# dwave-examples/image-generation

Hardware: AMD Instinct MI355X
Metric: DVAE+GRBM train-step images/s (MNIST) at 1/2/4/8 MI355X; loss parity vs CPU (higher is better)
Workload: dtype f32

## Files before the change

### image-generation_amd/csrc/special.hip

```cpp
#include <cstdlib>
#include "kernels.h"
#include "conv.h"

namespace dvg {

typedef float f32x16c __attribute__((ext_vector_type(16)));
__global__ __launch_bounds__(256) void enc_conv0_fwd_kernel(const float* __restrict__ img, int64_t B,
                                                            const float* __restrict__ w, const float* __restrict__ bias,
                                                            float* __restrict__ Y, float* __restrict__ stats_part) {
  __shared__ double red[2 * 4 * 32];
  const int tid = threadIdx.x, lane = tid & 63, wave = tid >> 6, hh = lane >> 5, c = lane & 31;
  float bw[5];
  int dy[5], dx[5];
#pragma unroll
  for (int j = 0; j < 5; ++j) {
    const int t = 2 * j + hh;
    bw[j] = t < 9 ? w[c * 9 + t] : bias[c];
    dy[j] = t < 9 ? t / 3 - 1 : 0;
    dx[j] = t < 9 ? t % 3 - 1 : 0;
  }
  const int64_t tiles = B * 32;
  double s1 = 0.0, s2 = 0.0;
  constexpr int TU = 2;
  for (int64_t t0 = ((int64_t)blockIdx.x * 4 + wave) * TU; t0 < tiles; t0 += (int64_t)gridDim.x * 4 * TU) {
// ... 345 lines not shown
  DVG_LAUNCH(K_BN_FINALIZE, enc_l0_moments_finalize_kernel, dim3(1), dim3(1024), 0, s, (const double*)part, nblk,
             (double)B * 1024.0, w, bias, mom, mean, invstd, rm, rv, nbt);
  return DVG_OK;
}

__global__ __launch_bounds__(320) void enc_l0_combine_kernel(const float* __restrict__ tot, const double* __restrict__ mom,
                                                             const float* __restrict__ wgt, const float* __restrict__ bias,
                                                             const float* __restrict__ mean, const float* __restrict__ gamma,
                                                             const float* __restrict__ invstd, double M,
                                                             float* __restrict__ gw, float* __restrict__ gb,
                                                             float* __restrict__ g_bn_b, float* __restrict__ g_bn_g) {
  const int w = threadIdx.x;
  const int co = w < 288 ? w / 9 : w - 288, t = w < 288 ? w % 9 : 9;
  const float sum_dz = tot[288 + co], sum_dzzh = tot[320 + co];
  const double m1 = (double)sum_dz / M, m2 = (double)sum_dzzh / M;
  const double shift = (double)bias[co] - (double)mean[co];
  double t1, t2 = 0.0;
  if (t < 9) {
    t1 = mom[t];
    for (int u = 0; u < 9; ++u) t2 += (double)wgt[co * 9 + u] * mom[u <= t ? enc_l0_pair_index(u, t) : enc_l0_pair_index(t, u)];
    t2 += shift * mom[t];
  } else {
    t1 = M;
    for (int u = 0; u < 9; ++u) t2 += (double)wgt[co * 9 + u] * mom[u];
    t2 += shift * M;
  }
  t2 *= (double)invstd[co];
  const float v = (float)((double)gamma[co] * (double)invstd[co] * ((double)tot[w] - m1 * t1 - m2 * t2));
  if (w < 288) gw[w] = v;
  else { gb[co] = v; g_bn_b[co] = sum_dz; g_bn_g[co] = sum_dzzh; }
}

int launch_enc_l0_combine(const float* tot, const double* mom, const float* w, const float* bias, const float* mean,
                          const float* gamma, const float* invstd, int64_t B, float* gw, float* gb, float* g_bn_b,
                          float* g_bn_g, hipStream_t s) {
  DVG_LAUNCH(K_MISC, enc_l0_combine_kernel, dim3(1), dim3(320), 0, s, tot, mom, w, bias, mean, gamma, invstd, (double)B * 1024.0,
             gw, gb, g_bn_b, g_bn_g);
  return DVG_OK;
}

typedef float f32x16s __attribute__((ext_vector_type(16)));
__global__ __launch_bounds__(256) void enc_conv0_wgrad_kernel(const float* __restrict__ img, int64_t B,
                                                              const float* __restrict__ dY, float* __restrict__ part) {
  __shared__ float red[4 * 32 * 33];
  const int tid = threadIdx.x, lane = tid & 63, wave = tid >> 6, hh = lane >> 5, c = lane & 31;
  const int64_t P = B * 1024;
  int64_t per = (P + gridDim.x * 4 - 1) / (gridDim.x * 4);
  per = (per + 1) & ~(int64_t)1;
  const int64_t p0 = ((int64_t)blockIdx.x * 4 + wave) * per;
  const int64_t p1 = p0 + per < P ? p0 + per : P;
  const int dy = c < 9 ? c / 3 - 1 : 0, dx = c < 9 ? c % 3 - 1 : 0;
  f32x16s acc = {0};
  constexpr int UN = 8;
  for (int64_t p = p0; p < p1; p += 2 * UN) {
    float av[UN], bv[UN];
    bool al[UN], bl[UN];
#pragma unroll
    for (int u = 0; u < UN; ++u) {
      const int64_t m = p + 2 * u + hh;
      const bool live = m < p1;
      const int64_t mc = live ? m : p0;
      av[u] = dY[mc * 32 + c];
      const uint32_t q = (uint32_t)(mc & 1023);
      const int yy = (int)morton_y(q) + dy, xx = (int)morton_x(q) + dx;
      const bool inb = yy >= 0 && yy < 32 && xx >= 0 && xx < 32;
      bv[u] = img[(mc >> 10) * 1024 + (inb ? yy * 32 + xx : 0)];
      al[u] = live;
      bl[u] = live && c < 9 && inb;
    }
#pragma unroll
    for (int u = 0; u < UN; ++u) {
      const float a = al[u] ? av[u] : 0.f;
      const float b = (c == 9) ? (al[u] ? 1.0f : 0.0f) : (bl[u] ? bv[u] : 0.f);
      acc = __builtin_amdgcn_mfma_f32_32x32x2f32(a, b, acc, 0, 0, 0);
    }
  }
#pragma unroll
  for (int r = 0; r < 16; ++r) red[(wave * 32 + (r & 3) + 8 * (r >> 2) + 4 * hh) * 33 + c] = acc[r];
  __syncthreads();
  for (int w = tid; w < 320; w += 256) {
    const int co = w < 288 ? w / 9 : w - 288, t = w < 288 ? w % 9 : 9;
    part[(size_t)blockIdx.x * 320 + w] =
        (red[(0 * 32 + co) * 33 + t] + red[(1 * 32 + co) * 33 + t]) + (red[(2 * 32 + co) * 33 + t] + red[(3 * 32 + co) * 33 + t]);
  }
}

int launch_enc_conv0_wgrad(const float* images, int64_t B, const float* dY, float* part, hipStream_t s) {
  DVG_LAUNCH(K_ENC_CONV0_WGRAD, enc_conv0_wgrad_kernel, dim3((unsigned)stream_blocks(8 * B)), dim3(256), 0, s, images, B, dY, part);
  return DVG_OK;
}

__global__ __launch_bounds__(256) void enc_proj_fwd_kernel(const float* __restrict__ P, int64_t B, int n,
                                                           const float* __restrict__ w, const float* __restrict__ b,
                                                           float* __restrict__ logits) {
  const int64_t total = B * n;
  const float w0 = w[0], w1 = w[1], w2 = w[2], w3 = w[3], bb = b[0];
  for (int64_t e = (int64_t)blockIdx.x * 256 + threadIdx.x; e < total; e += (int64_t)gridDim.x * 256) {
    const int c = (int)(e % n);
    const float* p = P + (e / n) * 4 * n + c;
    logits[e] = fmaf(p[3 * (size_t)n], w3, fmaf(p[2 * (size_t)n], w2, fmaf(p[n], w1, p[0] * w0))) + bb;
  }
}

int launch_enc_proj_fwd(const float* P, int64_t B, int n, const float* w, const float* b, float* logits, hipStream_t s) {
  const int64_t g = ceil_div(B * n, 256);
  DVG_LAUNCH(K_ENC_PROJ_FWD, enc_proj_fwd_kernel, dim3((unsigned)(g > 2048 ? 2048 : g)), dim3(256), 0, s, P, B, n, w, b,
             logits);
  return DVG_OK;
}

__global__ __launch_bounds__(256) void enc_proj_bwd_kernel(const float* __restrict__ P, int64_t B, int n,
                                                           const float* __restrict__ w, const float* __restrict__ dl,
                                                           float* __restrict__ dP, float* __restrict__ part) {
  __shared__ float red[5 * 256];
  const int n4 = n >> 2;
  const int64_t total = B * n4;
  const float wv[4] = {w[0], w[1], w[2], w[3]};
  float acc[5] = {0.f, 0.f, 0.f, 0.f, 0.f};
  for (int64_t e = (int64_t)blockIdx.x * 256 + threadIdx.x; e < total; e += (int64_t)gridDim.x * 256) {
    const int c4 = (int)(e % n4);
    const int64_t b = e / n4;
    const float4 g = *reinterpret_cast<const float4*>(dl + b * n + 4 * c4);
    const float* p = P + b * 4 * n + 4 * c4;
    float* dp = dP + b * 4 * n + 4 * c4;
    float4 pv[4];
#pragma unroll
    for (int k = 0; k < 4; ++k) pv[k] = *reinterpret_cast<const float4*>(p + (size_t)k * n);
#pragma unroll
    for (int k = 0; k < 4; ++k) {
      acc[k] = fmaf(g.x, pv[k].x, acc[k]);
      acc[k] = fmaf(g.y, pv[k].y, acc[k]);
      acc[k] = fmaf(g.z, pv[k].z, acc[k]);
      acc[k] = fmaf(g.w, pv[k].w, acc[k]);
      *reinterpret_cast<float4*>(dp + (size_t)k * n) = make_float4(g.x * wv[k], g.y * wv[k], g.z * wv[k], g.w * wv[k]);
    }
    acc[4] += g.x; acc[4] += g.y; acc[4] += g.z; acc[4] += g.w;
  }
#pragma unroll
  for (int k = 0; k < 5; ++k) red[k * 256 + threadIdx.x] = acc[k];
  __syncthreads();
  if (threadIdx.x < 5) {
    float t = 0.f;
    for (int j = 0; j < 256; ++j) t += red[threadIdx.x * 256 + j];
    part[(size_t)blockIdx.x * 5 + threadIdx.x] = t;
  }
}

int launch_enc_proj_bwd(const float* P, int64_t B, int n, const float* w, const float* dlogits, float* dP, float* part,
                        hipStream_t s) {
  DVG_LAUNCH(K_ENC_PROJ_BWD, enc_proj_bwd_kernel, dim3(EW_BLOCKS), dim3(256), 0, s, P, B, n, w, dlogits, dP, part);
  return DVG_OK;
}

template <bool ACT>
__global__ __launch_bounds__(256) void dec_conv3_fwd_kernel(const float* __restrict__ X, DecActIn in, int64_t N,
                                                            const float* __restrict__ w, const float* __restrict__ bias,
                                                            float* __restrict__ Y, float* __restrict__ stats_part) {
  constexpr int XP = 36;
  __shared__ __align__(16) float xs[64 * XP];
  __shared__ float w9[288];
  __shared__ __align__(16) float wfs[512];
  __shared__ float outs[256];
  __shared__ double red[2 * 4];
  const int tid = threadIdx.x, lane = tid & 63;
  const int cls = __builtin_amdgcn_readfirstlane(tid >> 6), pa = cls >> 1, pb = cls & 1;
  for (int i = tid; i < 288; i += 256) w9[i] = w[i];
  __syncthreads();
  for (int e = tid; e < 512; e += 256) {
    const int ci = e & 31, t = (e >> 5) & 3, cc = e >> 7;
    const int dr = t >> 1, dc = t & 1, qa = cc >> 1, qb = cc & 1;
    float acc = 0.f;
#pragma unroll
    for (int r = 0; r < 3; ++r)
#pragma unroll
      for (int sx = 0; sx < 3; ++sx)
        if (fold_src(qa, r) == dr && fold_src(qb, sx) == dc) acc += w9[ci * 9 + (8 - (r * 3 + sx))];
    wfs[e] = acc;
  }
  __syncthreads();
  const float* wcls = wfs + cls * 128;
  const float b0 = bias[0];
  const int ys = (int)morton_y((uint32_t)lane), xq = (int)morton_x((uint32_t)lane);
  int src[4];
#pragma unroll
  for (int t = 0; t < 4; ++t) {
    const int yy = ys - 1 + pa + (t >> 1), xx = xq - 1 + pb + (t & 1);
    src[t] = (yy >= 0 && yy < 8 && xx >= 0 && xx < 8) ? (int)morton((uint32_t)yy, (uint32_t)xx) : -1;
  }
  double s1 = 0.0, s2 = 0.0;
  const int cg4 = (tid & 7) * 4;
  float4 amu = {0.f, 0.f, 0.f, 0.f}, ais = amu, agm = amu, abt = amu;
  if (ACT) {
    amu = *reinterpret_cast<const float4*>(in.mean + cg4); ais = *reinterpret_cast<const float4*>(in.invstd + cg4);
    agm = *reinterpret_cast<const float4*>(in.gamma + cg4); abt = *reinterpret_cast<const float4*>(in.beta + cg4);
  }
  float4 nv[2], nmk = {1.f, 1.f, 1.f, 1.f};
  auto fetch = [&](int64_t img) {
    const int64_t im = img < N ? img : N - 1;
    const float4* g = reinterpret_cast<const float4*>((ACT ? in.y : X) + im * 64 * 32);
    nv[0] = g[tid]; nv[1] = g[tid + 256];
    if (ACT && in.mask) nmk = *reinterpret_cast<const float4*>(in.mask + im * 32 + cg4);
  };
  fetch(blockIdx.x);
  for (int64_t img = blockIdx.x; img < N; img += gridDim.x) {
    __syncthreads();
    {
      float4 mk = nmk;
      const float4 cv[2] = {nv[0], nv[1]};
      if (ACT && in.mask) {
        const float ks = 1.0f / DROPOUT_KEEP;
        mk.x *= ks; mk.y *= ks; mk.z *= ks; mk.w *= ks;
      }
      fetch(img + gridDim.x);
#pragma unroll
      for (int k = 0; k < 2; ++k) {
        const int e = tid + 256 * k;
        float4 v = cv[k];
        if (ACT) {
          float z;
          z = fmaf((v.x - amu.x) * ais.x, agm.x, abt.x); if (in.mask) z *= mk.x; v.x = z < 0.f ? z * LRELU_SLOPE : z;
          z = fmaf((v.y - amu.y) * ais.y, agm.y, abt.y); if (in.mask) z *= mk.y; v.y = z < 0.f ? z * LRELU_SLOPE : z;
          z = fmaf((v.z - amu.z) * ais.z, agm.z, abt.z); if (in.mask) z *= mk.z; v.z = z < 0.f ? z * LRELU_SLOPE : z;
          z = fmaf((v.w - amu.w) * ais.w, agm.w, abt.w); if (in.mask) z *= mk.w; v.w = z < 0.f ? z * LRELU_SLOPE : z;
        }
        *reinterpret_cast<float4*>(xs + (e >> 3) * XP + (e & 7) * 4) = v;
      }
    }
    __syncthreads();
    float acc = b0;
#pragma unroll
    for (int t = 0; t < 4; ++t) {
      if (src[t] >= 0) {
        const float4* row = reinterpret_cast<const float4*>(xs + src[t] * XP);
        const float4* wr = reinterpret_cast<const float4*>(wcls + t * 32);
#pragma unroll
        for (int k = 0; k < 8; ++k) {
          const float4 a = row[k], wv = wr[k];
          acc = fmaf(a.x, wv.x, acc); acc = fmaf(a.y, wv.y, acc);
          acc = fmaf(a.z, wv.z, acc); acc = fmaf(a.w, wv.w, acc);
        }
      }
    }
    outs[4 * lane + cls] = acc;
    s1 += (double)acc;
    s2 = fma((double)acc, (double)acc, s2);
    __syncthreads();
    Y[img * 256 + tid] = outs[tid];
  }
#pragma unroll
  for (int off = 32; off > 0; off >>= 1) { s1 += __shfl_xor(s1, off, 64); s2 += __shfl_xor(s2, off, 64); }
  if (lane == 0) { red[cls] = s1; red[4 + cls] = s2; }
  __syncthreads();
  if (tid == 0) {
    stats_part[(size_t)blockIdx.x * 2] = (float)((red[0] + red[1]) + (red[2] + red[3]));
    stats_part[(size_t)blockIdx.x * 2 + 1] = (float)((red[4] + red[5]) + (red[6] + red[7]));
  }
}

int dec_conv3_blocks(int64_t N) { return (int)(N < special_block_cap() ? N : special_block_cap()); }

int launch_dec_conv3_fwd(const float* X, int64_t N, const float* w, const float* b, float* Y, float* stats_part,
                         hipStream_t s) {
  DVG_LAUNCH(K_DEC_CONV3_FWD, dec_conv3_fwd_kernel<false>, dim3((unsigned)dec_conv3_blocks(N)), dim3(256), 0, s, X, DecActIn{}, N,
             w, b, Y, stats_part);
  return DVG_OK;
}

int launch_dec_conv3_fwd_act(const DecActIn& in, int64_t N, const float* w, const float* b, float* Y, float* stats_part,
                             hipStream_t s) {
  DVG_LAUNCH(K_DEC_CONV3_FWD, dec_conv3_fwd_kernel<true>, dim3((unsigned)dec_conv3_blocks(N)), dim3(256), 0, s, nullptr, in, N,
             w, b, Y, stats_part);
  return DVG_OK;
}


__global__ __launch_bounds__(288) void dec_conv3_bwd_kernel(const float* __restrict__ X, int64_t N,
                                                            const float* __restrict__ dY, const float* __restrict__ w,
                                                            float* __restrict__ dX, float* __restrict__ part) {
  __shared__ float dys[256];
  __shared__ float G[64 * 9];
  __shared__ __align__(16) float xs[64 * 32];
  __shared__ float ws[9 * 32];
  const int tid = threadIdx.x;
  for (int i = tid; i < 288; i += 288) ws[(i % 9) * 32 + i / 9] = w[i];
  int gsrc[2][4];
#pragma unroll
  for (int k = 0; k < 2; ++k) {
    const int e = tid + 288 * k, q = e / 9, t = e % 9, kh = t / 3, kw = t % 3;
    const int ys = (int)morton_y((uint32_t)q), xq = (int)morton_x((uint32_t)q);
#pragma unroll
    for (int u = 0; u < 4; ++u) {
      const int y = 2 * ys + (u >> 1) - 1 + kh, x = 2 * xq + (u & 1) - 1 + kw;
      gsrc[k][u] = (y >= 0 && y < 16 && x >= 0 && x < 16) ? (int)morton((uint32_t)y, (uint32_t)x) : -1;
    }
  }
  const int tap = tid >> 5, ci = tid & 31;
  const int q = tid >> 2, cg = (tid & 3) * 8;
  float acc = 0.f;
  __syncthreads();
  for (int64_t img = blockIdx.x; img < N; img += gridDim.x) {
    __syncthreads();
    if (tid < 256) dys[tid] = dY[img * 256 + tid];
    {
      const float4* g4 = reinterpret_cast<const float4*>(X + img * 64 * 32);
      for (int e = tid; e < 512; e += 288) reinterpret_cast<float4*>(xs)[e] = g4[e];
    }
    __syncthreads();
#pragma unroll
    for (int k = 0; k < 2; ++k) {
      float g = 0.f;
#pragma unroll
      for (int u = 0; u < 4; ++u) g += gsrc[k][u] >= 0 ? dys[gsrc[k][u]] : 0.f;
      G[tid + 288 * k] = g;
    }
    __syncthreads();
    if (tid < 256) {
      float o[8] = {0.f, 0.f, 0.f, 0.f, 0.f, 0.f, 0.f, 0.f};
#pragma unroll
      for (int t = 0; t < 9; ++t) {
        const float g = G[q * 9 + t];
        const float* wr = ws + t * 32 + cg;
#pragma unroll
        for (int k = 0; k < 8; ++k) o[k] = fmaf(g, wr[k], o[k]);
      }
      float4* dst = reinterpret_cast<float4*>(dX + (img * 64 + q) * 32 + cg);
      dst[0] = make_float4(o[0], o[1], o[2], o[3]);
      dst[1] = make_float4(o[4], o[5], o[6], o[7]);
    }
#pragma unroll 8
    for (int qq = 0; qq < 64; ++qq) acc = fmaf(G[qq * 9 + tap], xs[qq * 32 + ci], acc);
  }
  part[(size_t)blockIdx.x * 288 + tid] = acc;
}

int launch_dec_conv3_bwd(const float* X, int64_t N, const float* dY, const float* w, float* dX, float* part, hipStream_t s) {
  DVG_LAUNCH(K_DEC_CONV3_BWD, dec_conv3_bwd_kernel, dim3((unsigned)stream_blocks(N)), dim3(288), 0, s, X, N, dY, w, dX, part);
  return DVG_OK;
}


template <bool APPLY>
__global__ __launch_bounds__(256) void dec_conv3_bwd_fused_kernel(DecActIn in, int64_t N, const float* __restrict__ dY3,
                                                                  const float* __restrict__ w,
                                                                  const float* __restrict__ sum_dz,
                                                                  const float* __restrict__ sum_dzzh, float inv_m,
                                                                  float* __restrict__ dY2, float* __restrict__ part_w,
                                                                  float* __restrict__ part_bn) {
  __shared__ float dys[256];
  __shared__ float G[64 * 9];
  __shared__ __align__(16) float xs[APPLY ? 4 : 64 * 32];
  __shared__ float ws[9 * 32];
  __shared__ float red[8 * 32 * (APPLY ? 1 : 2)];
  const int tid = threadIdx.x;
  for (int i = tid; i < 288; i += 256) ws[(i % 9) * 32 + i / 9] = w[i];
  int gsrc[3][4];
#pragma unroll
  for (int k = 0; k < 3; ++k) {
    const int e = tid + 256 * k < 576 ? tid + 256 * k : 0, q = e / 9, t = e % 9, kh = t / 3, kw = t % 3;
    const int ys = (int)morton_y((uint32_t)q), xq = (int)morton_x((uint32_t)q);
#pragma unroll
    for (int u = 0; u < 4; ++u) {
      const int y = 2 * ys + (u >> 1) - 1 + kh, x = 2 * xq + (u & 1) - 1 + kw;
      gsrc[k][u] = (y >= 0 && y < 16 && x >= 0 && x < 16) ? (int)morton((uint32_t)y, (uint32_t)x) : -1;
    }
  }
  const int q = tid >> 2, cg = (tid & 3) * 8;
  const int lane = tid & 63, wv = tid >> 6, mt = lane & 15, mq = lane >> 4;
  f32x4c wacc[2] = {{0.f, 0.f, 0.f, 0.f}, {0.f, 0.f, 0.f, 0.f}};
  constexpr bool dg = true;
  __shared__ __align__(16) float cst[7][32];
  if (tid < 32) {
    cst[0][tid] = in.mean[tid]; cst[1][tid] = in.invstd[tid]; cst[2][tid] = in.gamma[tid]; cst[3][tid] = in.beta[tid];
    cst[4][tid] = in.gamma[tid] * in.invstd[tid];
    cst[5][tid] = APPLY ? sum_dz[tid] * inv_m : 0.f;
    cst[6][tid] = APPLY ? sum_dzzh[tid] * inv_m : 0.f;
  }
  float a1[8], a2[8];
#pragma unroll
  for (int k = 0; k < 8; ++k) { a1[k] = 0.f; a2[k] = 0.f; }
  const float ks = 1.0f / DROPOUT_KEEP;
  __syncthreads();
  float4 ny0 = {0.f, 0.f, 0.f, 0.f}, ny1 = ny0, nk0 = {1.f, 1.f, 1.f, 1.f}, nk1 = nk0;
  float ndy = 0.f;
  auto fetch = [&](int64_t img) {
    if (!dg) return;
    const int64_t im = img < N ? img : N - 1;
    const float4* yp = reinterpret_cast<const float4*>(in.y + (im * 64 + q) * 32 + cg);
    ny0 = yp[0]; ny1 = yp[1];
    if (in.mask) {
      const float4* mp = reinterpret_cast<const float4*>(in.mask + im * 32 + cg);
      nk0 = mp[0]; nk1 = mp[1];
    }
    ndy = dY3[im * 256 + tid];
  };
  fetch(blockIdx.x);
  for (int64_t img = blockIdx.x; img < N; img += gridDim.x) {
    __syncthreads();
    if (dg) dys[tid] = ndy;
    float zh[8], sl[8];
    const float4 y0 = ny0, y1 = ny1, k0 = nk0, k1 = nk1;
    fetch(img + gridDim.x);
    if (dg) {
      const float yv[8] = {y0.x, y0.y, y0.z, y0.w, y1.x, y1.y, y1.z, y1.w};
      const float kv[8] = {k0.x, k0.y, k0.z, k0.w, k1.x, k1.y, k1.z, k1.w};
      float xv[8];
#pragma unroll
      for (int k = 0; k < 8; ++k) {
        zh[k] = (yv[k] - cst[0][cg + k]) * cst[1][cg + k];
        float z = fmaf(zh[k], cst[2][cg + k], cst[3][cg + k]);
        const float mk = in.mask ? kv[k] * ks : 1.0f;
        if (in.mask) z *= mk;
        xv[k] = z < 0.f ? z * LRELU_SLOPE : z;
        sl[k] = ((xv[k] > 0.f) ? 1.0f : LRELU_SLOPE) * mk;
      }
      if (!APPLY) {
        float4* xd = reinterpret_cast<float4*>(xs + q * 32 + cg);
        xd[0] = make_float4(xv[0], xv[1], xv[2], xv[3]);
        xd[1] = make_float4(xv[4], xv[5], xv[6], xv[7]);
      }
    }
    __syncthreads();
#pragma unroll
    for (int k = 0; k < 3; ++k) {
      float g = 0.f;
#pragma unroll
      for (int u = 0; u < 4; ++u) g += gsrc[k][u] >= 0 ? dys[gsrc[k][u]] : 0.f;
      if (tid + 256 * k < 576) G[tid + 256 * k] = g;
    }
    __syncthreads();
    if (dg) {
      float o[8] = {0.f, 0.f, 0.f, 0.f, 0.f, 0.f, 0.f, 0.f};
#pragma unroll
      for (int t = 0; t < 9; ++t) {
        const float g = G[q * 9 + t];
        const float* wr = ws + t * 32 + cg;
#pragma unroll
        for (int k = 0; k < 8; ++k) o[k] = fmaf(g, wr[k], o[k]);
      }
      float v[8];
#pragma unroll
      for (int k = 0; k < 8; ++k) {
        const float dz = o[k] * sl[k];
        if (APPLY) {
          v[k] = cst[4][cg + k] * (dz - cst[5][cg + k] - zh[k] * cst[6][cg + k]);
          a1[k] += v[k];
        } else {
          a1[k] += dz;
          a2[k] = fmaf(dz, zh[k], a2[k]);
        }
      }
      if (APPLY) {
        float4* dst = reinterpret_cast<float4*>(dY2 + (img * 64 + q) * 32 + cg);
        dst[0] = make_float4(v[0], v[1], v[2], v[3]);
        dst[1] = make_float4(v[4], v[5], v[6], v[7]);
      }
    }
    if constexpr (!APPLY) {
      float av[4], b0[4], b1[4];
#pragma unroll
      for (int s4 = 0; s4 < 4; ++s4) {
        const int qq = 16 * wv + 4 * s4 + mq;
        av[s4] = G[qq * 9 + (mt < 9 ? mt : 0)];
        b0[s4] = xs[qq * 32 + mt];
        b1[s4] = xs[qq * 32 + 16 + mt];
      }
#pragma unroll
      for (int s4 = 0; s4 < 4; ++s4) {
        const float a_ = mt < 9 ? av[s4] : 0.f;
        wacc[0] = __builtin_amdgcn_mfma_f32_16x16x4f32(a_, b0[s4], wacc[0], 0, 0, 0);
        wacc[1] = __builtin_amdgcn_mfma_f32_16x16x4f32(a_, b1[s4], wacc[1], 0, 0, 0);
      }
    }
  }
  if constexpr (!APPLY) {
    __syncthreads();
    {
#pragma unroll
      for (int r = 0; r < 4; ++r) {
        const int row = 4 * mq + r;
        if (row < 9) {
          xs[(wv * 9 + row) * 32 + mt] = wacc[0][r];
          xs[(wv * 9 + row) * 32 + 16 + mt] = wacc[1][r];
        }
      }
    }
    __syncthreads();
    for (int e = tid; e < 288; e += 256)
      part_w[(size_t)blockIdx.x * 288 + e] = (xs[0 * 288 + e] + xs[1 * 288 + e]) + (xs[2 * 288 + e] + xs[3 * 288 + e]);
  }
  if (dg) {
#pragma unroll
    for (int k = 0; k < 8; ++k) {
#pragma unroll
      for (int off = 4; off < 64; off <<= 1) {
        a1[k] += __shfl_xor(a1[k], off, 64);
        if (!APPLY) a2[k] += __shfl_xor(a2[k], off, 64);
      }
    }
    if ((tid & 63) < 4) {
      const int wv = tid >> 6;
#pragma unroll
      for (int k = 0; k < 8; ++k) {
        red[(wv * 32 + cg + k) * (APPLY ? 1 : 2)] = a1[k];
        if (!APPLY) red[(wv * 32 + cg + k) * 2 + 1] = a2[k];
      }
    }
  }
  __syncthreads();
  if (APPLY) {
    if (tid < 32) part_bn[(size_t)blockIdx.x * 32 + tid] = (red[tid] + red[32 + tid]) + (red[64 + tid] + red[96 + tid]);
  } else if (tid < 64) {
    const int k = tid >> 5, cc = tid & 31;
    part_bn[(size_t)blockIdx.x * 64 + tid] =
        (red[(0 * 32 + cc) * 2 + k] + red[(1 * 32 + cc) * 2 + k]) + (red[(2 * 32 + cc) * 2 + k] + red[(3 * 32 + cc) * 2 + k]);
  }
}

int dec_tail_blocks(int64_t N) { return stream_blocks(N); }

int launch_dec_conv3_bwd_reduce(const DecActIn& in, int64_t N, const float* dY3, const float* w, float* part_w, float* part_bn,
                                hipStream_t s) {
  DVG_LAUNCH(K_DEC_CONV3_BWD, dec_conv3_bwd_fused_kernel<false>, dim3((unsigned)dec_tail_blocks(N)), dim3(256), 0, s, in, N, dY3,
             w, nullptr, nullptr, 0.f, nullptr, part_w, part_bn);
  return DVG_OK;
}

int launch_dec_conv3_bwd_apply(const DecActIn& in, int64_t N, const float* dY3, const float* w, const float* sum_dz,
                               const float* sum_dzzh, float* dY2, float* part_db, hipStream_t s) {
  DVG_LAUNCH(K_DEC_BN_ACT_BWD_APPLY, dec_conv3_bwd_fused_kernel<true>, dim3((unsigned)dec_tail_blocks(N)), dim3(256), 0, s, in, N,
             dY3, w, sum_dz, sum_dzzh, (float)(1.0 / ((double)N * 64.0)), dY2, nullptr, part_db);
  return DVG_OK;
}

__device__ __forceinline__ float dec_act1(float y, float mu, float is, float gm, float bt, const float* mask, int64_t img) {
  float z = fmaf((y - mu) * is, gm, bt);
  if (mask) z *= mask[img] * (1.0f / DROPOUT_KEEP);
  return z < 0.f ? z * LRELU_SLOPE : z;
}

template <bool ACT>
__global__ __launch_bounds__(256) void dec_final_fwd_kernel(const float* __restrict__ X, DecActIn in, int64_t N,
                                                            const float* __restrict__ w, const float* __restrict__ bias,
                                                            float* __restrict__ out) {
  __shared__ float xs[18 * 18];
  const float mu = ACT ? in.mean[0] : 0.f, is = ACT ? in.invstd[0] : 0.f, gm = ACT ? in.gamma[0] : 0.f, bt = ACT ? in.beta[0] : 0.f;
  const int tid = threadIdx.x;
  float wv[9];
#pragma unroll
  for (int t = 0; t < 9; ++t) wv[t] = w[t];
  const float bb = bias[0];
  for (int e = tid; e < 18 * 18; e += 256) xs[e] = 0.f;
  const int sy_ = (int)morton_y((uint32_t)tid), sx_ = (int)morton_x((uint32_t)tid);
  const int y = tid >> 3, x0 = (tid & 7) * 4;
  for (int64_t img = blockIdx.x; img < N; img += gridDim.x) {
    __syncthreads();
    xs[(sy_ + 1) * 18 + sx_ + 1] = ACT ? dec_act1(in.y[img * 256 + tid], mu, is, gm, bt, in.mask, img) : X[img * 256 + tid];
    __syncthreads();
    float acc[4] = {bb, bb, bb, bb};
#pragma unroll
    for (int kh = 0; kh < 3; ++kh) {
      const float* row = xs + (((y + 1 - kh) >> 1) + 1) * 18 + (x0 >> 1);
      const float v0 = row[0], v1 = row[1], v2 = row[2], v3 = row[3];
      const float src[6] = {v0, v1, v1, v2, v2, v3};
#pragma unroll
      for (int j = 0; j < 4; ++j)
#pragma unroll
        for (int kw = 0; kw < 3; ++kw) acc[j] = fmaf(src[j + 2 - kw], wv[kh * 3 + kw], acc[j]);
    }
    *reinterpret_cast<float4*>(out + img * 1024 + y * 32 + x0) = make_float4(acc[0], acc[1], acc[2], acc[3]);
  }
}

int launch_dec_final_fwd(const float* X, int64_t N, const float* w, const float* b, float* out, hipStream_t s) {
  DVG_LAUNCH(K_DEC_FINAL_FWD, dec_final_fwd_kernel<false>, dim3((unsigned)(N > 2048 ? 2048 : N)), dim3(256), 0, s, X, DecActIn{},
             N, w, b, out);
  return DVG_OK;
}

int launch_dec_final_fwd_act(const DecActIn& in, int64_t N, const float* w, const float* b, float* out, hipStream_t s) {
  DVG_LAUNCH(K_DEC_FINAL_FWD, dec_final_fwd_kernel<true>, dim3((unsigned)(N > 2048 ? 2048 : N)), dim3(256), 0, s, nullptr, in, N,
             w, b, out);
  return DVG_OK;
}

template <int MODE>
__global__ __launch_bounds__(256) void dec_final_dgrad_kernel(const float* __restrict__ dOut, int64_t N,
                                                              const float* __restrict__ w, float* __restrict__ dX,
                                                              DecActIn in, const float* __restrict__ sum_dz,
                                                              const float* __restrict__ sum_dzzh, float inv_m,
                                                              float* __restrict__ part) {
  constexpr bool BN = MODE != 0;
  __shared__ float gs[34 * 34];
  __shared__ float red[2 * 4];
  float r1 = 0.f, r2 = 0.f;
  const float mu = BN ? in.mean[0] : 0.f, is = BN ? in.invstd[0] : 0.f, gm = BN ? in.gamma[0] : 0.f, bt = BN ? in.beta[0] : 0.f;
  const float m1 = MODE == 2 ? sum_dz[0] * inv_m : 0.f, m2 = MODE == 2 ? sum_dzzh[0] * inv_m : 0.f, gi = gm * is;
  const int tid = threadIdx.x;
  float wf[4][4];
#pragma unroll
  for (int u = 0; u < 4; ++u)
#pragma unroll
    for (int v = 0; v < 4; ++v) {
      float acc = 0.f;
#pragma unroll
      for (int kh = 0; kh < 3; ++kh)
#pragma unroll
        for (int kw = 0; kw < 3; ++kw) {
          const int sy = (u - 1) - (kh - 1), sx = (v - 1) - (kw - 1);
          if (sy >= 0 && sy < 2 && sx >= 0 && sx < 2) acc += w[kh * 3 + kw];
        }
      wf[u][v] = acc;
    }
  for (int e = tid; e < 34 * 34; e += 256) gs[e] = 0.f;
  const int ys = (int)morton_y((uint32_t)tid), xq = (int)morton_x((uint32_t)tid);
  for (int64_t img = blockIdx.x; img < N; img += gridDim.x) {
    __syncthreads();
    {
      const float4 v = reinterpret_cast<const float4*>(dOut + img * 1024)[tid];
      float* d = gs + ((tid >> 3) + 1) * 34 + (tid & 7) * 4 + 1;
      d[0] = v.x; d[1] = v.y; d[2] = v.z; d[3] = v.w;
    }
    __syncthreads();
    float acc = 0.f;
#pragma unroll
    for (int u = 0; u < 4; ++u) {
      const float* row = gs + (2 * ys + u) * 34 + 2 * xq;
#pragma unroll
      for (int v = 0; v < 4; ++v) acc = fmaf(row[v], wf[u][v], acc);
    }
    if (MODE == 0) dX[img * 256 + tid] = acc;
    if (BN) {
      const float zh = (in.y[img * 256 + tid] - mu) * is;
      const float mk = in.mask ? in.mask[img] * (1.0f / DROPOUT_KEEP) : 1.0f;
      const float dz = acc * ((fmaf(zh, gm, bt) > 0.f) ? 1.0f : LRELU_SLOPE) * mk;
      if (MODE == 1) {
        r1 += dz;
        r2 = fmaf(dz, zh, r2);
      } else {
        const float v = gi * (dz - m1 - zh * m2);
        dX[img * 256 + tid] = v;
        r1 += v;
      }
    }
  }
  if (BN) {
#pragma unroll
    for (int off = 32; off > 0; off >>= 1) { r1 += __shfl_xor(r1, off, 64); r2 += __shfl_xor(r2, off, 64); }
    if ((tid & 63) == 0) { red[tid >> 6] = r1; red[4 + (tid >> 6)] = r2; }
    __syncthreads();
    if (MODE == 1 && tid < 2) part[(size_t)blockIdx.x * 2 + tid] = (red[4 * tid] + red[4 * tid + 1]) + (red[4 * tid + 2] + red[4 * tid + 3]);
    if (MODE == 2 && tid == 0) part[blockIdx.x] = (red[0] + red[1]) + (red[2] + red[3]);
  }
}

int dec_final_dgrad_blocks(int64_t N) { return (int)(N > 2048 ? 2048 : N); }

int launch_dec_final_dgrad(const float* dOut, int64_t N, const float* w, float* dX, hipStream_t s) {
  DVG_LAUNCH(K_DEC_FINAL_BWD, dec_final_dgrad_kernel<0>, dim3((unsigned)dec_final_dgrad_blocks(N)), dim3(256), 0, s, dOut, N, w,
             dX, DecActIn{}, nullptr, nullptr, 0.f, nullptr);
  return DVG_OK;
}

int launch_dec_final_dgrad_bn(const float* dOut, int64_t N, const float* w, const DecActIn& in, float* part, hipStream_t s) {
  DVG_LAUNCH(K_DEC_FINAL_BWD, dec_final_dgrad_kernel<1>, dim3((unsigned)dec_final_dgrad_blocks(N)), dim3(256), 0, s, dOut, N, w,
             nullptr, in, nullptr, nullptr, 0.f, part);
  return DVG_OK;
}

int launch_dec_final_dgrad_apply(const float* dOut, int64_t N, const float* w, const DecActIn& in, const float* sum_dz,
                                 const float* sum_dzzh, float* dY, float* part_db, hipStream_t s) {
  DVG_LAUNCH(K_DEC_FINAL_BWD, dec_final_dgrad_kernel<2>, dim3((unsigned)dec_final_dgrad_blocks(N)), dim3(256), 0, s, dOut,
             N, w, dY, in, sum_dz, sum_dzzh, (float)(1.0 / ((double)N * 256.0)), part_db);
  return DVG_OK;
}

template <int MODE>
__global__ __launch_bounds__(256) void dec_tail_mse_kernel(DecActIn in, int64_t N, const float* __restrict__ w,
                                                           const float* __restrict__ bias, const float* __restrict__ images,
                                                           int R, float gscale, const float* __restrict__ sum_dz,
                                                           const float* __restrict__ sum_dzzh, float inv_m,
                                                           float* __restrict__ dY, float* __restrict__ part,
                                                           double* __restrict__ mse_part) {
  __shared__ float xs[18 * 18];
  __shared__ float gs[34 * 34];
  __shared__ float red[2 * 4];
  __shared__ double redd[4];
  const int tid = threadIdx.x;
  const float mu = in.mean[0], is = in.invstd[0], gm = in.gamma[0], bt = in.beta[0];
  const float m1 = MODE == 2 ? sum_dz[0] * inv_m : 0.f, m2 = MODE == 2 ? sum_dzzh[0] * inv_m : 0.f, gi = gm * is;
  float wv[9];
#pragma unroll
  for (int t = 0; t < 9; ++t) wv[t] = w[t];
  const float bb = bias[0];
  float wf[4][4];
#pragma unroll
  for (int u = 0; u < 4; ++u)
#pragma unroll
    for (int v = 0; v < 4; ++v) {
      float acc = 0.f;
#pragma unroll
      for (int kh = 0; kh < 3; ++kh)
#pragma unroll
        for (int kw = 0; kw < 3; ++kw) {
          const int sy = (u - 1) - (kh - 1), sx = (v - 1) - (kw - 1);
          if (sy >= 0 && sy < 2 && sx >= 0 && sx < 2) acc += w[kh * 3 + kw];
        }
      wf[u][v] = acc;
    }
  for (int e = tid; e < 18 * 18; e += 256) xs[e] = 0.f;
  for (int e = tid; e < 34 * 34; e += 256) gs[e] = 0.f;
  const int ys = (int)morton_y((uint32_t)tid), xq = (int)morton_x((uint32_t)tid);
  const int y = tid >> 3, x0 = (tid & 7) * 4;
  float r1 = 0.f, r2 = 0.f;
  double msum = 0.0;
  float nyv = 0.f, nmk = 1.0f;
  float4 ntv = {0.f, 0.f, 0.f, 0.f};
  auto fetch = [&](int64_t img) {
    const int64_t im = img < N ? img : N - 1;
    nyv = in.y[im * 256 + tid];
    ntv = *reinterpret_cast<const float4*>(images + (im / R) * 1024 + y * 32 + x0);
    if (in.mask) nmk = in.mask[im];
  };
  fetch(blockIdx.x);
  for (int64_t img = blockIdx.x; img < N; img += gridDim.x) {
    __syncthreads();
    const float yv = nyv, mkv = nmk;
    const float4 tv = ntv;
    fetch(img + gridDim.x);
    {
      float z = fmaf((yv - mu) * is, gm, bt);
      if (in.mask) z *= mkv * (1.0f / DROPOUT_KEEP);
      xs[(ys + 1) * 18 + xq + 1] = z < 0.f ? z * LRELU_SLOPE : z;
    }
    __syncthreads();
    float acc[4] = {bb, bb, bb, bb};
#pragma unroll
    for (int kh = 0; kh < 3; ++kh) {
      const float* row = xs + (((y + 1 - kh) >> 1) + 1) * 18 + (x0 >> 1);
      const float v0 = row[0], v1 = row[1], v2 = row[2], v3 = row[3];
      const float src[6] = {v0, v1, v1, v2, v2, v3};
#pragma unroll
      for (int j = 0; j < 4; ++j)
#pragma unroll
        for (int kw = 0; kw < 3; ++kw) acc[j] = fmaf(src[j + 2 - kw], wv[kh * 3 + kw], acc[j]);
    }
    const float d0 = acc[0] - tv.x, d1 = acc[1] - tv.y, d2 = acc[2] - tv.z, d3 = acc[3] - tv.w;
    if (MODE == 1) msum += (double)(d0 * d0) + (double)(d1 * d1) + (double)(d2 * d2) + (double)(d3 * d3);
    float* gd = gs + (y + 1) * 34 + x0 + 1;
    gd[0] = gscale * d0; gd[1] = gscale * d1; gd[2] = gscale * d2; gd[3] = gscale * d3;
    __syncthreads();
    float dx = 0.f;
#pragma unroll
    for (int u = 0; u < 4; ++u) {
      const float* row = gs + (2 * ys + u) * 34 + 2 * xq;
#pragma unroll
      for (int v = 0; v < 4; ++v) dx = fmaf(row[v], wf[u][v], dx);
    }
    const float zh = (yv - mu) * is;
    const float mk = in.mask ? mkv * (1.0f / DROPOUT_KEEP) : 1.0f;
    const float dz = dx * ((fmaf(zh, gm, bt) > 0.f) ? 1.0f : LRELU_SLOPE) * mk;
    if (MODE == 1) {
      r1 += dz;
      r2 = fmaf(dz, zh, r2);
    } else {
      const float v = gi * (dz - m1 - zh * m2);
      dY[img * 256 + tid] = v;
      r1 += v;
    }
  }
#pragma unroll
  for (int off = 32; off > 0; off >>= 1) { r1 += __shfl_xor(r1, off, 64); r2 += __shfl_xor(r2, off, 64); msum += __shfl_xor(msum, off, 64); }
  if ((tid & 63) == 0) { red[tid >> 6] = r1; red[4 + (tid >> 6)] = r2; redd[tid >> 6] = msum; }
  __syncthreads();
  if (MODE == 1 && tid < 2) part[(size_t)blockIdx.x * 2 + tid] = (red[4 * tid] + red[4 * tid + 1]) + (red[4 * tid + 2] + red[4 * tid + 3]);
  if (MODE == 2 && tid == 0) part[blockIdx.x] = (red[0] + red[1]) + (red[2] + red[3]);
  if (MODE == 1 && tid == 0) mse_part[blockIdx.x] = (redd[0] + redd[1]) + (redd[2] + redd[3]);
}

int launch_dec_tail_mse_sums(const DecActIn& in, int64_t N, const float* w, const float* bias, const float* images, int R,
                             float gscale, float* part, double* mse_part, hipStream_t s) {
  DVG_LAUNCH(K_DEC_FINAL_FWD, dec_tail_mse_kernel<1>, dim3((unsigned)dec_final_dgrad_blocks(N)), dim3(256), 0, s, in, N, w, bias,
             images, R, gscale, nullptr, nullptr, 0.f, nullptr, part, mse_part);
  return DVG_OK;
}

int launch_dec_tail_mse_apply(const DecActIn& in, int64_t N, const float* w, const float* bias, const float* images, int R,
                              float gscale, const float* sum_dz, const float* sum_dzzh, float* dY, float* part_db,
                              hipStream_t s) {
  DVG_LAUNCH(K_DEC_FINAL_BWD, dec_tail_mse_kernel<2>, dim3((unsigned)dec_final_dgrad_blocks(N)), dim3(256), 0, s, in, N, w, bias,
             images, R, gscale, sum_dz, sum_dzzh, (float)(1.0 / ((double)N * 256.0)), dY, part_db, nullptr);
  return DVG_OK;
}

template <bool ACT, bool MSE>
__global__ __launch_bounds__(256) void dec_final_wgrad_kernel(const float* __restrict__ X, DecActIn in, int64_t N,
                                                              const float* __restrict__ dOut, float* __restrict__ part,
                                                              const float* __restrict__ w, const float* __restrict__ bias,
                                                              const float* __restrict__ images, int R, float gscale) {
  __shared__ float Xs[2][18 * 18];
  float wv[9];
#pragma unroll
  for (int t = 0; t < 9; ++t) wv[t] = MSE ? w[t] : 0.f;
  const float bb = MSE ? bias[0] : 0.f;
  const float mu = ACT ? in.mean[0] : 0.f, is = ACT ? in.invstd[0] : 0.f, gm = ACT ? in.gamma[0] : 0.f, bt = ACT ? in.beta[0] : 0.f;
  __shared__ float red[10 * 256];
  const int tid = threadIdx.x;
  for (int e = tid; e < 2 * 18 * 18; e += 256) (&Xs[0][0])[e] = 0.f;
  __syncthreads();
  const int spos = ((int)morton_y((uint32_t)tid) + 1) * 18 + (int)morton_x((uint32_t)tid) + 1;
  const int i = tid >> 4, j = tid & 15;
  float acc[10];
#pragma unroll
  for (int k = 0; k < 10; ++k) acc[k] = 0.f;
  int64_t img = blockIdx.x;
  float xv = 0.f;
  float2 g0 = {0.f, 0.f}, g1 = {0.f, 0.f};
  const float* gsrc = MSE ? images : dOut;
  if (img < N) {
    xv = ACT ? dec_act1(in.y[img * 256 + tid], mu, is, gm, bt, in.mask, img) : X[img * 256 + tid];
    const int64_t gi_ = MSE ? img / R : img;
    g0 = *reinterpret_cast<const float2*>(gsrc + gi_ * 1024 + (2 * i) * 32 + 2 * j);
    g1 = *reinterpret_cast<const float2*>(gsrc + gi_ * 1024 + (2 * i + 1) * 32 + 2 * j);
  }
  for (int buf = 0; img < N; img += gridDim.x, buf ^= 1) {
    Xs[buf][spos] = xv;
    float g[2][2] = {{g0.x, g0.y}, {g1.x, g1.y}};
    const int64_t nimg = img + gridDim.x;
    if (nimg < N) {
      xv = ACT ? dec_act1(in.y[nimg * 256 + tid], mu, is, gm, bt, in.mask, nimg) : X[nimg * 256 + tid];
      const int64_t gi_ = MSE ? nimg / R : nimg;
      g0 = *reinterpret_cast<const float2*>(gsrc + gi_ * 1024 + (2 * i) * 32 + 2 * j);
      g1 = *reinterpret_cast<const float2*>(gsrc + gi_ * 1024 + (2 * i + 1) * 32 + 2 * j);
    }
    __syncthreads();
    float sn[3][3];
#pragma unroll
    for (int r = 0; r < 3; ++r)
#pragma unroll
      for (int c = 0; c < 3; ++c) sn[r][c] = Xs[buf][(i + r) * 18 + j + c];
    if (MSE) {
#pragma unroll
      for (int a = 0; a < 2; ++a)
#pragma unroll
        for (int b = 0; b < 2; ++b) {
          float rec = bb;
#pragma unroll
          for (int kh = 0; kh < 3; ++kh)
#pragma unroll
            for (int kw = 0; kw < 3; ++kw) {
              const int r = a == 0 ? (kh == 2 ? 0 : 1) : (kh == 0 ? 2 : 1);
              const int c = b == 0 ? (kw == 2 ? 0 : 1) : (kw == 0 ? 2 : 1);
              rec = fmaf(sn[r][c], wv[kh * 3 + kw], rec);
            }
          g[a][b] = gscale * (rec - g[a][b]);
        }
    }
#pragma unroll
    for (int a = 0; a < 2; ++a)
#pragma unroll
      for (int b = 0; b < 2; ++b) {
#pragma unroll
        for (int kh = 0; kh < 3; ++kh)
#pragma unroll
          for (int kw = 0; kw < 3; ++kw) {
            const int r = a == 0 ? (kh == 2 ? 0 : 1) : (kh == 0 ? 2 : 1);
            const int c = b == 0 ? (kw == 2 ? 0 : 1) : (kw == 0 ? 2 : 1);
            acc[kh * 3 + kw] = fmaf(g[a][b], sn[r][c], acc[kh * 3 + kw]);
          }
        acc[9] += g[a][b];
      }
  }
#pragma unroll
  for (int k = 0; k < 10; ++k) red[k * 256 + tid] = acc[k];
  __syncthreads();
// ... 28 lines not shown
```

Measured before the change: 589,200.

## Deepen prefetch pipeline in decoder conv3 kernels and drop per-image division

```diff
diff --git a/image-generation_amd/csrc/special.hip b/image-generation_amd/csrc/special.hip
--- a/image-generation_amd/csrc/special.hip
+++ b/image-generation_amd/csrc/special.hip
@@ -521,7 +521,7 @@
   return DVG_OK;
 }
 
-template <bool ACT>
+template <bool ACT, int LA>
 __global__ __launch_bounds__(256) void dec_conv3_fwd_kernel(const float* __restrict__ X, DecActIn in, int64_t N,
                                                             const float* __restrict__ w, const float* __restrict__ bias,
                                                             float* __restrict__ Y, float* __restrict__ stats_part) {
@@ -563,59 +563,71 @@
     amu = *reinterpret_cast<const float4*>(in.mean + cg4); ais = *reinterpret_cast<const float4*>(in.invstd + cg4);
     agm = *reinterpret_cast<const float4*>(in.gamma + cg4); abt = *reinterpret_cast<const float4*>(in.beta + cg4);
   }
-  float4 nv[2], nmk = {1.f, 1.f, 1.f, 1.f};
-  auto fetch = [&](int64_t img) {
+  float4 nv[LA][2], nmk[LA];
+  auto fetch = [&](int u, int64_t img) {
     const int64_t im = img < N ? img : N - 1;
     const float4* g = reinterpret_cast<const float4*>((ACT ? in.y : X) + im * 64 * 32);
-    nv[0] = g[tid]; nv[1] = g[tid + 256];
-    if (ACT && in.mask) nmk = *reinterpret_cast<const float4*>(in.mask + im * 32 + cg4);
+    nv[u][0] = g[tid]; nv[u][1] = g[tid + 256];
+    nmk[u] = make_float4(1.f, 1.f, 1.f, 1.f);
+    if (ACT) nmk[u] = *reinterpret_cast<const float4*>(in.mask ? in.mask + im * 32 + cg4 : in.mean + cg4);
   };
-  fetch(blockIdx.x);
-  for (int64_t img = blockIdx.x; img < N; img += gridDim.x) {
-    __syncthreads();
-    {
-      float4 mk = nmk;
-      const float4 cv[2] = {nv[0], nv[1]};
-      if (ACT && in.mask) {
-        const float ks = 1.0f / DROPOUT_KEEP;
-        mk.x *= ks; mk.y *= ks; mk.z *= ks; mk.w *= ks;
-      }
-      fetch(img + gridDim.x);
-#pragma unroll
-      for (int k = 0; k < 2; ++k) {
-        const int e = tid + 256 * k;
-        float4 v = cv[k];
-        if (ACT) {
-          float z;
-          z = fmaf((v.x - amu.x) * ais.x, agm.x, abt.x); if (in.mask) z *= mk.x; v.x = z < 0.f ? z * LRELU_SLOPE : z;
-          z = fmaf((v.y - amu.y) * ais.y, agm.y, abt.y); if (in.mask) z *= mk.y; v.y = z < 0.f ? z * LRELU_SLOPE : z;
-          z = fmaf((v.z - amu.z) * ais.z, agm.z, abt.z); if (in.mask) z *= mk.z; v.z = z < 0.f ? z * LRELU_SLOPE : z;
-          z = fmaf((v.w - amu.w) * ais.w, agm.w, abt.w); if (in.mask) z *= mk.w; v.w = z < 0.f ? z * LRELU_SLOPE : z;
-        }
-        *reinterpret_cast<float4*>(xs + (e >> 3) * XP + (e & 7) * 4) = v;
-      }
-    }
-    __syncthreads();
-    float acc = b0;
-#pragma unroll
-    for (int t = 0; t < 4; ++t) {
-      if (src[t] >= 0) {
-        const float4* row = reinterpret_cast<const float4*>(xs + src[t] * XP);
-        const float4* wr = reinterpret_cast<const float4*>(wcls + t * 32);
-#pragma unroll
-        for (int k = 0; k < 8; ++k) {
-          const float4 a = row[k], wv = wr[k];
-          acc = fmaf(a.x, wv.x, acc); acc = fmaf(a.y, wv.y, acc);
-          acc = fmaf(a.z, wv.z, acc); acc = fmaf(a.w, wv.w, acc);
-        }
-      }
-    }
-    outs[4 * lane + cls] = acc;
-    s1 += (double)acc;
-    s2 = fma((double)acc, (double)acc, s2);
-    __syncthreads();
-    Y[img * 256 + tid] = outs[tid];
-  }
+#pragma unroll
+  for (int u = 0; u < LA; ++u) {
+    fetch(u, blockIdx.x + (int64_t)u * gridDim.x);
+    __builtin_amdgcn_sched_barrier(0);
+  }
+  [&] {
+  for (int64_t img0 = blockIdx.x; img0 < N; img0 += (int64_t)LA * gridDim.x) {
+#pragma unroll
+    for (int u = 0; u < LA; ++u) {
+      const int64_t img = img0 + (int64_t)u * gridDim.x;
+      if (img >= N) return;
+      __syncthreads();
+      {
+        float4 mk = nmk[u];
+        const float4 cv[2] = {nv[u][0], nv[u][1]};
+        if (ACT && in.mask) {
+          const float ks = 1.0f / DROPOUT_KEEP;
+          mk.x *= ks; mk.y *= ks; mk.z *= ks; mk.w *= ks;
+        }
+#pragma unroll
+        for (int k = 0; k < 2; ++k) {
+          const int e = tid + 256 * k;
+          float4 v = cv[k];
+          if (ACT) {
+            float z;
+            z = fmaf((v.x - amu.x) * ais.x, agm.x, abt.x); if (in.mask) z *= mk.x; v.x = z < 0.f ? z * LRELU_SLOPE : z;
+            z = fmaf((v.y - amu.y) * ais.y, agm.y, abt.y); if (in.mask) z *= mk.y; v.y = z < 0.f ? z * LRELU_SLOPE : z;
+            z = fmaf((v.z - amu.z) * ais.z, agm.z, abt.z); if (in.mask) z *= mk.z; v.z = z < 0.f ? z * LRELU_SLOPE : z;
+            z = fmaf((v.w - amu.w) * ais.w, agm.w, abt.w); if (in.mask) z *= mk.w; v.w = z < 0.f ? z * LRELU_SLOPE : z;
+          }
+          *reinterpret_cast<float4*>(xs + (e >> 3) * XP + (e & 7) * 4) = v;
+        }
+        fetch(u, img + (int64_t)LA * gridDim.x);
+      }
+      __syncthreads();
+      float acc = b0;
+#pragma unroll
+      for (int t = 0; t < 4; ++t) {
+        if (src[t] >= 0) {
+          const float4* row = reinterpret_cast<const float4*>(xs + src[t] * XP);
+          const float4* wr = reinterpret_cast<const float4*>(wcls + t * 32);
+#pragma unroll
+          for (int k = 0; k < 8; ++k) {
+            const float4 a = row[k], wv = wr[k];
+            acc = fmaf(a.x, wv.x, acc); acc = fmaf(a.y, wv.y, acc);
+            acc = fmaf(a.z, wv.z, acc); acc = fmaf(a.w, wv.w, acc);
+          }
+        }
+      }
+      outs[4 * lane + cls] = acc;
+      s1 += (double)acc;
+      s2 = fma((double)acc, (double)acc, s2);
+      __syncthreads();
+      Y[img * 256 + tid] = outs[tid];
+    }
+  }
+  }();
 #pragma unroll
   for (int off = 32; off > 0; off >>= 1) { s1 += __shfl_xor(s1, off, 64); s2 += __shfl_xor(s2, off, 64); }
   if (lane == 0) { red[cls] = s1; red[4 + cls] = s2; }
@@ -626,18 +638,23 @@
   }
 }
 
+#ifndef DVG_DEC_TAIL_LA
+#define DVG_DEC_TAIL_LA 2
+#endif
+constexpr int DEC_TAIL_LA = DVG_DEC_TAIL_LA;
+
 int dec_conv3_blocks(int64_t N) { return (int)(N < special_block_cap() ? N : special_block_cap()); }
 
 int launch_dec_conv3_fwd(const float* X, int64_t N, const float* w, const float* b, float* Y, float* stats_part,
                          hipStream_t s) {
-  DVG_LAUNCH(K_DEC_CONV3_FWD, dec_conv3_fwd_kernel<false>, dim3((unsigned)dec_conv3_blocks(N)), dim3(256), 0, s, X, DecActIn{}, N,
+  DVG_LAUNCH(K_DEC_CONV3_FWD, (dec_conv3_fwd_kernel<false, DEC_TAIL_LA>), dim3((unsigned)dec_conv3_blocks(N)), dim3(256), 0, s, X, DecActIn{}, N,
              w, b, Y, stats_part);
   return DVG_OK;
 }
 
 int launch_dec_conv3_fwd_act(const DecActIn& in, int64_t N, const float* w, const float* b, float* Y, float* stats_part,
                              hipStream_t s) {
-  DVG_LAUNCH(K_DEC_CONV3_FWD, dec_conv3_fwd_kernel<true>, dim3((unsigned)dec_conv3_blocks(N)), dim3(256), 0, s, nullptr, in, N,
+  DVG_LAUNCH(K_DEC_CONV3_FWD, (dec_conv3_fwd_kernel<true, DEC_TAIL_LA>), dim3((unsigned)dec_conv3_blocks(N)), dim3(256), 0, s, nullptr, in, N,
              w, b, Y, stats_part);
   return DVG_OK;
 }
@@ -708,7 +725,7 @@
 }
 
 
-template <bool APPLY>
+template <bool APPLY, int LA>
 __global__ __launch_bounds__(256) void dec_conv3_bwd_fused_kernel(DecActIn in, int64_t N, const float* __restrict__ dY3,
                                                                   const float* __restrict__ w,
                                                                   const float* __restrict__ sum_dz,
@@ -749,95 +766,116 @@
   for (int k = 0; k < 8; ++k) { a1[k] = 0.f; a2[k] = 0.f; }
   const float ks = 1.0f / DROPOUT_KEEP;
   __syncthreads();
-  float4 ny0 = {0.f, 0.f, 0.f, 0.f}, ny1 = ny0, nk0 = {1.f, 1.f, 1.f, 1.f}, nk1 = nk0;
-  float ndy = 0.f;
-  auto fetch = [&](int64_t img) {
+  constexpr bool MASK_LDS = LA > 1;
+  __shared__ __align__(16) float mks[MASK_LDS ? 32 : 4];
+  float4 ny0[LA], ny1[LA], nk0 = {1.f, 1.f, 1.f, 1.f}, nk1 = nk0;
+  float ndy[LA], nmk[LA];
+  auto fetch = [&](int st, int64_t img) {
     if (!dg) return;
     const int64_t im = img < N ? img : N - 1;
+    if (in.mask) {
+      if (MASK_LDS) {
+        if (tid < 32) nmk[st] = in.mask[im * 32 + tid];
+      } else {
+        const float4* mp = reinterpret_cast<const float4*>(in.mask + im * 32 + cg);
+        nk0 = mp[0]; nk1 = mp[1];
+      }
+    }
     const float4* yp = reinterpret_cast<const float4*>(in.y + (im * 64 + q) * 32 + cg);
-    ny0 = yp[0]; ny1 = yp[1];
-    if (in.mask) {
-      const float4* mp = reinterpret_cast<const float4*>(in.mask + im * 32 + cg);
-      nk0 = mp[0]; nk1 = mp[1];
-    }
-    ndy = dY3[im * 256 + tid];
+    ny0[st] = yp[0]; ny1[st] = yp[1];
+    ndy[st] = dY3[im * 256 + tid];
   };
-  fetch(blockIdx.x);
-  for (int64_t img = blockIdx.x; img < N; img += gridDim.x) {
-    __syncthreads();
-    if (dg) dys[tid] = ndy;
-    float zh[8], sl[8];
-    const float4 y0 = ny0, y1 = ny1, k0 = nk0, k1 = nk1;
-    fetch(img + gridDim.x);
-    if (dg) {
-      const float yv[8] = {y0.x, y0.y, y0.z, y0.w, y1.x, y1.y, y1.z, y1.w};
-      const float kv[8] = {k0.x, k0.y, k0.z, k0.w, k1.x, k1.y, k1.z, k1.w};
-      float xv[8];
-#pragma unroll
-      for (int k = 0; k < 8; ++k) {
-        zh[k] = (yv[k] - cst[0][cg + k]) * cst[1][cg + k];
-        float z = fmaf(zh[k], cst[2][cg + k], cst[3][cg + k]);
-        const float mk = in.mask ? kv[k] * ks : 1.0f;
-        if (in.mask) z *= mk;
-        xv[k] = z < 0.f ? z * LRELU_SLOPE : z;
-        sl[k] = ((xv[k] > 0.f) ? 1.0f : LRELU_SLOPE) * mk;
-      }
-      if (!APPLY) {
-        float4* xd = reinterpret_cast<float4*>(xs + q * 32 + cg);
-        xd[0] = make_float4(xv[0], xv[1], xv[2], xv[3]);
-        xd[1] = make_float4(xv[4], xv[5], xv[6], xv[7]);
-      }
-    }
-    __syncthreads();
-#pragma unroll
-    for (int k = 0; k < 3; ++k) {
-      float g = 0.f;
-#pragma unroll
-      for (int u = 0; u < 4; ++u) g += gsrc[k][u] >= 0 ? dys[gsrc[k][u]] : 0.f;
-      if (tid + 256 * k < 576) G[tid + 256 * k] = g;
-    }
-    __syncthreads();
-    if (dg) {
-      float o[8] = {0.f, 0.f, 0.f, 0.f, 0.f, 0.f, 0.f, 0.f};
-#pragma unroll
-      for (int t = 0; t < 9; ++t) {
-        const float g = G[q * 9 + t];
-        const float* wr = ws + t * 32 + cg;
-#pragma unroll
-        for (int k = 0; k < 8; ++k) o[k] = fmaf(g, wr[k], o[k]);
-      }
-      float v[8];
-#pragma unroll
-      for (int k = 0; k < 8; ++k) {
-        const float dz = o[k] * sl[k];
+#pragma unroll
+  for (int st = 0; st < LA; ++st) {
+    nmk[st] = 1.f;
+    fetch(st, blockIdx.x + (int64_t)st * gridDim.x);
+    __builtin_amdgcn_sched_barrier(0);
+  }
+  if (MASK_LDS && tid < 32) mks[tid] = nmk[0];
+  for (int64_t img0 = blockIdx.x; img0 < N; img0 += (int64_t)LA * gridDim.x) {
+#pragma unroll
+    for (int st = 0; st < LA; ++st) {
+      const int64_t img = img0 + (int64_t)st * gridDim.x;
+      if (img >= N) break;
+      __syncthreads();
+      if (dg) dys[tid] = ndy[st];
+      float zh[8], sl[8];
+      const float4 y0 = ny0[st], y1 = ny1[st];
+      const float4 k0 = MASK_LDS ? *reinterpret_cast<const float4*>(mks + cg) : nk0;
+      const float4 k1 = MASK_LDS ? *reinterpret_cast<const float4*>(mks + cg + 4) : nk1;
+      if (LA == 1) fetch(st, img + (int64_t)LA * gridDim.x);
+      if (dg) {
+        const float yv[8] = {y0.x, y0.y, y0.z, y0.w, y1.x, y1.y, y1.z, y1.w};
+        const float kv[8] = {k0.x, k0.y, k0.z, k0.w, k1.x, k1.y, k1.z, k1.w};
+        float xv[8];
+#pragma unroll
+        for (int k = 0; k < 8; ++k) {
+          zh[k] = (yv[k] - cst[0][cg + k]) * cst[1][cg + k];
+          float z = fmaf(zh[k], cst[2][cg + k], cst[3][cg + k]);
+          const float mk = in.mask ? kv[k] * ks : 1.0f;
+          if (in.mask) z *= mk;
+          xv[k] = z < 0.f ? z * LRELU_SLOPE : z;
+          sl[k] = ((xv[k] > 0.f) ? 1.0f : LRELU_SLOPE) * mk;
+        }
+        if (!APPLY) {
+          float4* xd = reinterpret_cast<float4*>(xs + q * 32 + cg);
+          xd[0] = make_float4(xv[0], xv[1], xv[2], xv[3]);
+          xd[1] = make_float4(xv[4], xv[5], xv[6], xv[7]);
+        }
+      }
+      if (LA > 1) fetch(st, img + (int64_t)LA * gridDim.x);
+      __syncthreads();
+#pragma unroll
+      for (int k = 0; k < 3; ++k) {
+        float g = 0.f;
+#pragma unroll
+        for (int u = 0; u < 4; ++u) g += gsrc[k][u] >= 0 ? dys[gsrc[k][u]] : 0.f;
+        if (tid + 256 * k < 576) G[tid + 256 * k] = g;
+      }
+      __syncthreads();
+      if (MASK_LDS && in.mask && tid < 32) mks[tid] = nmk[(st + 1) % LA];
+      if (dg) {
+        float o[8] = {0.f, 0.f, 0.f, 0.f, 0.f, 0.f, 0.f, 0.f};
+#pragma unroll
+        for (int t = 0; t < 9; ++t) {
+          const float g = G[q * 9 + t];
+          const float* wr = ws + t * 32 + cg;
+#pragma unroll
+          for (int k = 0; k < 8; ++k) o[k] = fmaf(g, wr[k], o[k]);
+        }
+        float v[8];
+#pragma unroll
+        for (int k = 0; k < 8; ++k) {
+          const float dz = o[k] * sl[k];
+          if (APPLY) {
+            v[k] = cst[4][cg + k] * (dz - cst[5][cg + k] - zh[k] * cst[6][cg + k]);
+            a1[k] += v[k];
+          } else {
+            a1[k] += dz;
+            a2[k] = fmaf(dz, zh[k], a2[k]);
+          }
+        }
         if (APPLY) {
-          v[k] = cst[4][cg + k] * (dz - cst[5][cg + k] - zh[k] * cst[6][cg + k]);
-          a1[k] += v[k];
-        } else {
-          a1[k] += dz;
-          a2[k] = fmaf(dz, zh[k], a2[k]);
-        }
-      }
-      if (APPLY) {
-        float4* dst = reinterpret_cast<float4*>(dY2 + (img * 64 + q) * 32 + cg);
-        dst[0] = make_float4(v[0], v[1], v[2], v[3]);
-        dst[1] = make_float4(v[4], v[5], v[6], v[7]);
-      }
-    }
-    if constexpr (!APPLY) {
-      float av[4], b0[4], b1[4];
-#pragma unroll
-      for (int s4 = 0; s4 < 4; ++s4) {
-        const int qq = 16 * wv + 4 * s4 + mq;
-        av[s4] = G[qq * 9 + (mt < 9 ? mt : 0)];
-        b0[s4] = xs[qq * 32 + mt];
-        b1[s4] = xs[qq * 32 + 16 + mt];
-      }
-#pragma unroll
-      for (int s4 = 0; s4 < 4; ++s4) {
-        const float a_ = mt < 9 ? av[s4] : 0.f;
-        wacc[0] = __builtin_amdgcn_mfma_f32_16x16x4f32(a_, b0[s4], wacc[0], 0, 0, 0);
-        wacc[1] = __builtin_amdgcn_mfma_f32_16x16x4f32(a_, b1[s4], wacc[1], 0, 0, 0);
+          float4* dst = reinterpret_cast<float4*>(dY2 + (img * 64 + q) * 32 + cg);
+          dst[0] = make_float4(v[0], v[1], v[2], v[3]);
+          dst[1] = make_float4(v[4], v[5], v[6], v[7]);
+        }
+      }
+      if constexpr (!APPLY) {
+        float av[4], b0[4], b1[4];
+#pragma unroll
+        for (int s4 = 0; s4 < 4; ++s4) {
+          const int qq = 16 * wv + 4 * s4 + mq;
+          av[s4] = G[qq * 9 + (mt < 9 ? mt : 0)];
+          b0[s4] = xs[qq * 32 + mt];
+          b1[s4] = xs[qq * 32 + 16 + mt];
+        }
+#pragma unroll
+        for (int s4 = 0; s4 < 4; ++s4) {
+          const float a_ = mt < 9 ? av[s4] : 0.f;
+          wacc[0] = __builtin_amdgcn_mfma_f32_16x16x4f32(a_, b0[s4], wacc[0], 0, 0, 0);
+          wacc[1] = __builtin_amdgcn_mfma_f32_16x16x4f32(a_, b1[s4], wacc[1], 0, 0, 0);
+        }
       }
     }
   }
@@ -889,14 +927,14 @@
 
 int launch_dec_conv3_bwd_reduce(const DecActIn& in, int64_t N, const float* dY3, const float* w, float* part_w, float* part_bn,
                                 hipStream_t s) {
-  DVG_LAUNCH(K_DEC_CONV3_BWD, dec_conv3_bwd_fused_kernel<false>, dim3((unsigned)dec_tail_blocks(N)), dim3(256), 0, s, in, N, dY3,
+  DVG_LAUNCH(K_DEC_CONV3_BWD, (dec_conv3_bwd_fused_kernel<false, DEC_TAIL_LA>), dim3((unsigned)dec_tail_blocks(N)), dim3(256), 0, s, in, N, dY3,
              w, nullptr, nullptr, 0.f, nullptr, part_w, part_bn);
   return DVG_OK;
 }
 
 int launch_dec_conv3_bwd_apply(const DecActIn& in, int64_t N, const float* dY3, const float* w, const float* sum_dz,
                                const float* sum_dzzh, float* dY2, float* part_db, hipStream_t s) {
-  DVG_LAUNCH(K_DEC_BN_ACT_BWD_APPLY, dec_conv3_bwd_fused_kernel<true>, dim3((unsigned)dec_tail_blocks(N)), dim3(256), 0, s, in, N,
+  DVG_LAUNCH(K_DEC_BN_ACT_BWD_APPLY, (dec_conv3_bwd_fused_kernel<true, 1>), dim3((unsigned)dec_tail_blocks(N)), dim3(256), 0, s, in, N,
              dY3, w, sum_dz, sum_dzzh, (float)(1.0 / ((double)N * 64.0)), dY2, nullptr, part_db);
   return DVG_OK;
 }
@@ -1084,11 +1122,17 @@
   double msum = 0.0;
   float nyv = 0.f, nmk = 1.0f;
   float4 ntv = {0.f, 0.f, 0.f, 0.f};
+  const int64_t last_q = (N - 1) / R;
+  const int grid_q = (int)(gridDim.x / (unsigned)R), grid_r = (int)(gridDim.x % (unsigned)R);
+  int64_t row_q = (int64_t)(blockIdx.x / (unsigned)R);
+  int row_r = (int)(blockIdx.x % (unsigned)R);
   auto fetch = [&](int64_t img) {
     const int64_t im = img < N ? img : N - 1;
     nyv = in.y[im * 256 + tid];
-    ntv = *reinterpret_cast<const float4*>(images + (im / R) * 1024 + y * 32 + x0);
+    ntv = *reinterpret_cast<const float4*>(images + (img < N ? row_q : last_q) * 1024 + y * 32 + x0);
     if (in.mask) nmk = in.mask[im];
+    row_q += grid_q; row_r += grid_r;
+    if (row_r >= R) { row_r -= R; ++row_q; }
   };
   fetch(blockIdx.x);
   for (int64_t img = blockIdx.x; img < N; img += gridDim.x) {
```

Result: no change. 588,300 (median of 3 runs) (-0.1%).
